# xflouris/libpll-2

Measured on AMD Instinct MI355X. Metric: M site-CLV-updates/s, higher is better.
Workload: dtype f64; 1 GPU; 4-state DNA GTR+G4, 64-taxon balanced tree, 100k sites, tips set with pll_set_tip_states (device reads 1-byte codes: tip x tip / tip x inner kernels at the leaves); sites_per_gpu=100000, ops_per_traversal=62, states=4, taxa=64, step=pll_update_partials(full traversal) + pll_compute_edge_loglikelihood, driver=C loop over the two C-ABI calls (csrc/workload/step_loop.c), parallelism=1 GPU

## Files before the change

libpll-2_amd/csrc/hip/chain_plan.h:

```cpp
#pragma once
struct ChainLaunchRec
{
  unsigned first_head, nchains;
  unsigned variant;
};

struct ChainPlan
{
  std::vector<pllgpu_op_t> key;
  unsigned long long epoch = 0;
  unsigned entries = 0;
  std::vector<CCLaunch> cc;
  std::vector<CC16Launch> cc16;
  std::vector<ChainLaunchRec> stages;
  std::vector<ChainHead> heads;
  std::vector<ChainStepLoad> loads;
  std::vector<ChainStepOp> sops;
  std::vector<unsigned> head_top_clv;
  std::vector<int> head_top_scaler;
  std::vector<unsigned char> head_variant;
  bool in_kernarg = false;
  size_t held_from = 0;
  unsigned launches = 0;
  double bytes = 0.0;
  bool tree = false;
  TreeEnd tree_end[2];
  double tree_bytes = 0.0;
  std::vector<pllgpu_op_t> cherries;
};

static void drop_chain_plan(pllgpu_ctx *c)
{
  if (c->pending_plan == c->plan) c->pending_plan = nullptr;
  delete c->plan;
  c->plan = nullptr;
}

static void chain_steps_on_device(const pllgpu_ctx *c, const ChainPlan &pl, const ChainStepLoad *&lp, const ChainStepOp *&op)
{
  const unsigned char *base = c->chain_dev.p;
  const size_t heads_bytes = pl.heads.size() * sizeof(ChainHead), loads_bytes = pl.loads.size() * sizeof(ChainStepLoad);
  lp = reinterpret_cast<const ChainStepLoad *>(base + heads_bytes);
  op = reinterpret_cast<const ChainStepOp *>(base + heads_bytes + loads_bytes);
}

static void launch_chain_heads(pllgpu_ctx *c, const ChainPlan &pl, unsigned first_head, unsigned nchains, unsigned variant)
{
  const unsigned tiles = (pl.entries + 63) / 64;
  dim3 grid(tiles, nchains), block(256);
  if (pl.in_kernarg)
  {
// ... 11 lines not shown
    }
    with_chain_variant(c->gg.scale_mode, variant, [&](auto SMV, auto C0, auto S1, auto C1) {
      hipLaunchKernelGGL((k_partials_dna_chain_pack<SMV(), C0(), S1(), C1()>), grid, block, 0, c->stream, pack, pl.entries);
    });
  }
  else
  {
    const ChainHead *hp = reinterpret_cast<const ChainHead *>(c->chain_dev.p) + first_head;
    const ChainStepLoad *lp;
    const ChainStepOp *op;
    chain_steps_on_device(c, pl, lp, op);
    with_chain_variant(c->gg.scale_mode, variant, [&](auto SMV, auto C0, auto S1, auto C1) {
      hipLaunchKernelGGL((k_partials_dna_chain<SMV(), C0(), S1(), C1()>), grid, block, 0, c->stream, hp, lp, op, pl.entries);
    });
  }
}

static int launch_chain_plan(pllgpu_ctx *c, const ChainPlan &pl, bool hold)
{
  if (hold && pl.tree)
  {
    c->chain_held = c->tree_held = true;
    c->last_launches = 0;
    c->last_bytes = pl.tree_bytes;
    return 0;
  }
  for (const CC16Launch &l : pl.cc16)
    if (int rc = launch_cc16(c, l.pack, l.n, l.entries)) return rc;
  for (const CCLaunch &l : pl.cc)
    if (int rc = launch_cc(c, l.pack, l.n, l.entries, l.lk, CK_FCC)) return rc;
  const size_t upto = hold ? pl.held_from : pl.stages.size();
  for (size_t i = 0; i < upto; ++i) launch_chain_heads(c, pl, pl.stages[i].first_head, pl.stages[i].nchains, pl.stages[i].variant);
  c->chain_held = hold && upto < pl.stages.size();
  c->last_launches = pl.launches - (unsigned)(pl.stages.size() - upto);
  c->last_bytes = pl.bytes;
  return launch_status();
}

static int launch_held_tree_groups(pllgpu_ctx *c, bool lean = false)
{
  if (!c->tree_held || !c->plan) return 0;
  c->tree_held = false;
  const ChainPlan &pl = *c->plan;
  for (const CCLaunch &l : pl.cc)
    if (int rc = launch_cc(c, l.pack, l.n, l.entries, l.lk, CK_FCC, lean)) return rc;
  c->last_launches += (unsigned)pl.cc.size();
  c->last_bytes = pl.bytes;
// ... 180 lines not shown
        if (P.role[j] == Role::Plain && P.absorb[j] && P.pr_of[1 - P.acc_side[j]][j] == (int)i) st = P.chains[P.chain_of[j]].stage;
    if (stage) stage[i] = st;
    if (chain) chain[i] = member ? -1 : (P.form[i] == 2 ? -2 : P.chain_of[i]);
    if (form) form[i] = member ? 3 : P.form[i];
    stages = std::max(stages, st);
  }
  return (int)stages;
}

static bool use_cc16(const pllgpu_ctx *c, unsigned entries, unsigned count)
{
  if (c->fuse_cc16 >= 0) return c->fuse_cc16 != 0;
  return (size_t)entries * count >= (size_t)9000000;
}

constexpr unsigned kTreeMinEntries = 20000;
static bool use_tree(const pllgpu_ctx *c, unsigned entries, unsigned count)
{
  if (count != 62u || !c->defer_tail) return false;
  if (c->fuse_tree >= 0) return c->fuse_tree != 0;
  return entries >= kTreeMinEntries;
}

struct ChainBuild
{
  const pllgpu_op_t *ops;
  const ChainPartition &part;
  std::vector<DevOp> dev;
  unsigned entries, clv_bytes, sc_bytes;

  ChainLeaf leaf(unsigned i, int sd, bool &tip, ChainLeafBytes &lb) const
  {
    ChainLeaf l;
    tip = ops[i].flags & (sd ? PLLGPU_OP_RIGHT_TIP : PLLGPU_OP_LEFT_TIP);
    lb.clv = lb.aux = lb.pad = 0u;
    if (tip)
    {
      l.data = sd ? dev[i].rtip : dev[i].ltip;
      l.scaler = nullptr;
      lb.aux = (entries + 3u) & ~3u;
    }
    else
    {
      l.data = sd ? dev[i].right : dev[i].left;
      l.scaler = sd ? dev[i].rscaler : dev[i].lscaler;
      lb.clv = clv_bytes;
// ... 97 lines not shown
}

static void choose_held_stage(const pllgpu_ctx *c, ChainPlan *pl)
{
  if (pl->held_from == (size_t)-1) pl->held_from = pl->stages.size();
  unsigned held_chains = 0;
  for (size_t i = pl->held_from; i < pl->stages.size(); ++i) held_chains += pl->stages[i].nchains;
  if (held_chains > 2 || (c->geo.sites + 63) / 64 > 4096u) pl->held_from = pl->stages.size();
  unsigned tail_steps = 0, tail_heads = 0;
  for (size_t i = pl->held_from; i < pl->stages.size(); ++i)
    for (unsigned h = pl->stages[i].first_head; h < pl->stages[i].first_head + pl->stages[i].nchains; ++h, ++tail_heads)
      tail_steps += pl->heads[h].nsteps + 1;
  if (tail_heads && tail_steps + (2u - std::min(tail_heads, 2u)) > (unsigned)kChainPackSteps) pl->in_kernarg = false;
}

static void plan_tree(const pllgpu_ctx *c, const ChainBuild &b, unsigned count, ChainPlan *pl)
{
  const ChainPartition &part = b.part;
  const pllgpu_op_t *ops = b.ops;
  if (count != 62u || part.groups.size() != 8u || part.chains.size() != 2u || pl->heads.size() != 2u) return;
  if (pl->cc.size() != 1u || pl->cc[0].n != 8u || pl->cc[0].lk != CK_FCC || !pl->cc16.empty()) return;
  if (pl->held_from != 0 || pl->stages.empty()) return;
  std::vector<int> group_of(count, -1);
  for (size_t gi = 0; gi < 8u; ++gi)
  {
    const FusedGroup &g = part.groups[gi];
    if (g.lk != CK_FCC || g.rk != CK_FCC || g.absorbed) return;
    group_of[g.p] = (int)gi;
  }
  unsigned seen = 0;
  for (unsigned k = 0; k < 2u; ++k)
  {
    const unsigned top = part.chains[k].ops[0];
    unsigned h = 0;
    while (h < 2u && (pl->head_top_clv[h] != ops[top].parent_clv || pl->head_top_scaler[h] != ops[top].parent_scaler)) ++h;
    if (h == 2u) return;
    TreeEnd &end = pl->tree_end[h];
    memset(&end, 0, sizeof end);
    to_top(b.dev[top], end.top);
    for (int sd = 0; sd < 2; ++sd)
    {
      if (!part.is_chain_op(top, sd)) return;
      const unsigned mid = (unsigned)part.pr_of[sd][top];
      to_top(b.dev[mid], end.mid[sd]);
      for (int sd2 = 0; sd2 < 2; ++sd2)
      {
        const int pr = part.pr_of[sd2][mid];
        if (pr < 0 || group_of[pr] < 0) return;
        seen |= 1u << group_of[pr];
        end.g[sd * 2 + sd2] = pl->cc[0].pack.g[group_of[pr]];
      }
    }
  }
  if (seen != 0xffu) return;
  for (unsigned i = 0; i < count; ++i)
    if ((ops[i].flags & PLLGPU_OP_LEFT_TIP) && (ops[i].flags & PLLGPU_OP_RIGHT_TIP)) pl->cherries.push_back(ops[i]);
  if (pl->cherries.size() != 32u) return;
  for (unsigned i = 0; i < count; ++i)
  {
    const bool lt = (ops[i].flags & PLLGPU_OP_LEFT_TIP) != 0, rt = (ops[i].flags & PLLGPU_OP_RIGHT_TIP) != 0;
    pl->tree_bytes += (c->lazy_cherries && lt && rt) ? 2.0 * ops[i].parent_entries : op_traffic(c, ops[i], lt, rt);
  }
  pl->tree = true;
}

static int build_chain_plan(pllgpu_ctx *c, const pllgpu_op_t *ops, unsigned count, unsigned entries, ChainPartition &part, bool want_tree,
                            ChainPlan *pl)
{
  const std::vector<PChain> &chains = part.chains;
  ChainBuild b{ops, part, std::vector<DevOp>(count), entries, (unsigned)(clv_elems(c, entries) * sizeof(double)),
               entries * (c->gg.scale_mode == 2 ? 16u : 4u)};
  c->last_bytes = 0.0;
  for (unsigned i = 0; i < count; ++i)
    if (part.role[i] == Role::Plain)
      if (int rc = resolve_op(c, ops[i], b.dev[i])) return rc;
  sort_groups_by_level(part.groups);
  if (int rc = build_cc_launches(c, ops, part.groups, 0, part.groups.size(), pl->cc)) return rc;
  if (int rc = build_cc16_launches(c, ops, part.groups, pl->cc16)) return rc;
  unsigned max_stage = 0;
  for (const PChain &ch : chains) max_stage = std::max(max_stage, ch.stage);
  pl->entries = entries;
  pl->in_kernarg = true;
  pl->held_from = (size_t)-1;
  std::vector<unsigned> variant_of(chains.size());
// ... 81 lines not shown
```

libpll-2_amd/csrc/hip/kernels_dna.h:

```cpp
#pragma once
#include "kernels_common.h"

constexpr unsigned kDnaTile = 16 * 64;

template <bool TIP>
__device__ __forceinline__ void dna_fetch(double (&x)[4], const double *__restrict__ base, unsigned k, unsigned code)
{
  if (TIP)
  {
#pragma unroll
    for (int j = 0; j < 4; ++j) x[j] = (code >> j) & 1u ? 1.0 : 0.0;
  }
  else
  {
#pragma unroll
    for (int j = 0; j < 4; ++j) x[j] = __builtin_nontemporal_load(base + (k * 4 + j) * 64);
  }
}

typedef double dbl2 __attribute__((ext_vector_type(2)));
constexpr unsigned kAosLeft = 1u, kAosRight = 2u, kAosParent = 4u, kStreamLeft = 16u, kStreamRight = 32u;

struct DnaCoop
{
// ... 746 lines not shown
  FOp a, b;
  TOp aa, ab;
  TOp ba, bb;
};

constexpr int kMaxCCGroups = 9;

struct CCPack
{
  CCGroup g[kMaxCCGroups];
};

template <bool STORE = true>
__device__ __forceinline__ void dna_cherry(const TOp &t, size_t off, unsigned n, bool valid, int scale_mode, double (&v)[4][4], uint4 &sc)
{
  double xl[4][4], xr[4][4];
  dna_tip_rows(xl, t.ltip[n]);
  dna_tip_rows(xr, t.rtip[n]);
  int mode;
  dna_combine(t, scale_mode, xl, make_uint4(0, 0, 0, 0), xr, make_uint4(0, 0, 0, 0), v, sc, mode);
  if (STORE) dna_store<true>(t.parent, t.pscaler, off, n, valid, mode, v, sc);
}

template <int KIND, bool STORE_CHERRIES = true>
__device__ __forceinline__ void dna_cc_child(const FOp &pop, bool left_side, const FOp &cop, const TOp &x, const TOp &y, size_t off,
                                             unsigned n, bool valid, int scale_mode, double (&v)[4][4], uint4 &sc)
{
  if (KIND == CK_FCC)
  {
    double vx[4][4], vy[4][4];
    uint4 scx, scy;
    int mode;
    dna_cherry<STORE_CHERRIES>(x, off, n, valid, scale_mode, vx, scx);
    dna_cherry<STORE_CHERRIES>(y, off, n, valid, scale_mode, vy, scy);
    dna_combine(cop, scale_mode, vx, scx, vy, scy, v, sc, mode);
    dna_store<true>(cop.parent, cop.pscaler, off, n, valid, mode, v, sc);
  }
  else
  {
    DnaRaw raw;
    dna_child_load<KIND>(pop, left_side, cop, off, n, raw);
    dna_child_compute<KIND>(pop, left_side, cop, n, scale_mode, raw, v, sc);
  }
}

template <int LK, int RK, bool STORE_CHERRIES = true>
__global__ __launch_bounds__(256) void k_partials_dna_cc(const CCPack pack, unsigned entries, int scale_mode, unsigned tiles_per_wave,
                                                          unsigned stream_parent, unsigned nx, unsigned ny, unsigned xcd_order)
{
  unsigned bx, by;
  if (!xcd_block(nx, ny, xcd_order, bx, by)) return;
  const CCGroup &g = pack.g[by];
  for (unsigned t = 0; t < tiles_per_wave; ++t)
  {
    DnaTile w;
    if (!dna_tile(w, bx, tiles_per_wave, t, entries)) break;
    double va[4][4], vb[4][4], v[4][4];
    uint4 sca, scb, sc;
    int mode;
    dna_cc_child<LK, STORE_CHERRIES>(g.p, true, g.a, g.aa, g.ab, w.off, w.n, w.valid, scale_mode, va, sca);
    dna_cc_child<RK, STORE_CHERRIES>(g.p, false, g.b, g.ba, g.bb, w.off, w.n, w.valid, scale_mode, vb, scb);
    dna_combine(g.p, scale_mode, va, sca, vb, scb, v, sc, mode);
    dna_store_parent(stream_parent != 0, g.p.parent, g.p.pscaler, w.off, w.n, w.valid, mode, v, sc);
  }
}

constexpr int CK_F8 = 7;

struct CC16Group
{
  FOp p;
  CCGroup a, b;
};

constexpr int kMaxCC16Groups = 4;

struct CC16Pack
{
  CC16Group g[kMaxCC16Groups];
};

__device__ __forceinline__ void dna_cc8(const CCGroup &g, size_t off, unsigned n, bool valid, int scale_mode, double (&v)[4][4], uint4 &sc)
{
  double va[4][4], vb[4][4];
// ... 775 lines not shown
{
  TreeEnd end[2];
};
static_assert(sizeof(TreePack) + sizeof(DevEdge) + 12 <= 4000, "k_edge_dna_tree's arguments must fit the kernarg segment");

__device__ __forceinline__ void dna_tree_put(double (*xv)[64], uint4 *xs, unsigned lane, const double (&v)[4][4], uint4 sc)
{
#pragma unroll
  for (int k = 0; k < 4; ++k)
#pragma unroll
    for (int i = 0; i < 4; ++i) xv[k * 4 + i][lane] = v[k][i];
  xs[lane] = sc;
}

__device__ __forceinline__ void dna_tree_get(const double (*xv)[64], const uint4 *xs, unsigned lane, double (&v)[4][4], uint4 &sc)
{
#pragma unroll
  for (int k = 0; k < 4; ++k)
#pragma unroll
    for (int i = 0; i < 4; ++i) v[k][i] = xv[k * 4 + i][lane];
  sc = xs[lane];
}

template <bool STORE_CHERRIES>
__device__ __forceinline__ void dna_cc8_parked(const CCGroup &g, double (*xv)[64], uint4 *xs, unsigned lane, size_t off, unsigned n, bool valid,
                                               int scale_mode, double (&v)[4][4], uint4 &sc)
{
  double vb[4][4], u[4][4];
  uint4 scb, scu;
  int mode;
  dna_cc_child<CK_FCC, STORE_CHERRIES>(g.p, true, g.a, g.aa, g.ab, off, n, valid, scale_mode, v, sc);
  dna_tree_put(xv, xs, lane, v, sc);
  asm volatile("" ::: "memory");
  dna_cc_child<CK_FCC, STORE_CHERRIES>(g.p, false, g.b, g.ba, g.bb, off, n, valid, scale_mode, vb, scb);
  asm volatile("" ::: "memory");
  dna_tree_get(xv, xs, lane, v, sc);
  dna_combine(g.p, scale_mode, v, sc, vb, scb, u, scu, mode);
  dna_store<true>(g.p.parent, g.p.pscaler, off, n, valid, mode, u, scu);
#pragma unroll
  for (int k = 0; k < 4; ++k)
#pragma unroll
    for (int i = 0; i < 4; ++i) v[k][i] = u[k][i];
  sc = scu;
}

__device__ __forceinline__ void dna_tree_up(const TOp &op, const double (*xv)[64], const uint4 *xs, unsigned lane, size_t off, unsigned n, bool valid,
                                            int scale_mode, double (&v)[4][4], uint4 &sc)
{
  double vb[4][4], u[4][4];
  uint4 scb, scu;
  int mode;
  dna_tree_get(xv, xs, lane, vb, scb);
  dna_combine(op, scale_mode, v, sc, vb, scb, u, scu, mode);
  dna_store<true>(op.parent, op.pscaler, off, n, valid, mode, u, scu);
#pragma unroll
  for (int k = 0; k < 4; ++k)
#pragma unroll
    for (int i = 0; i < 4; ++i) v[k][i] = u[k][i];
  sc = scu;
}

template <bool STORE_CHERRIES>
__global__ __launch_bounds__(512) void k_edge_dna_tree(const DevEdge e, const TreePack pack, unsigned entries, int scale_mode, unsigned xcd_order)
{
  __shared__ double xv[8][16][64];
  __shared__ uint4 xs[8][64];
  __shared__ unsigned last;
  __shared__ double ws[4];
  const unsigned ntiles = (entries + 63u) / 64u;
  const unsigned tile = xcd_linear(ntiles, xcd_order);
  if (tile == ~0u) return;
  const unsigned lane = threadIdx.x & 63u;
  const unsigned wave = __builtin_amdgcn_readfirstlane(threadIdx.x >> 6);
  const unsigned n0 = tile * 64u + lane;
  const bool valid = n0 < entries;
  const unsigned n = valid ? n0 : entries - 1;
  const size_t off = (size_t)tile * kDnaTile + lane;
  const TreeEnd &end = pack.end[wave >> 2];
  double v[4][4];
  uint4 sc;
  dna_cc8_parked<STORE_CHERRIES>(end.g[wave & 3u], xv[wave], xs[wave], lane, off, n, valid, scale_mode, v, sc);
  if (wave & 1u) dna_tree_put(xv[wave], xs[wave], lane, v, sc);
  lds_barrier();
  if (wave & 1u) return;
  dna_tree_up(end.mid[(wave >> 1) & 1u], xv[wave + 1u], xs[wave + 1u], lane, off, n, valid, scale_mode, v, sc);
  if (wave & 2u) dna_tree_put(xv[wave], xs[wave], lane, v, sc);
  lds_barrier();
  if (!(wave & 2u)) dna_tree_up(end.top, xv[wave + 2u], xs[wave + 2u], lane, off, n, valid, scale_mode, v, sc);
  if (wave == 4u) dna_tree_put(xv[4], xs[4], lane, v, sc);
  lds_barrier();
  if (wave == 0u)
  {
    double vc[4][4];
    uint4 scc;
    dna_tree_get(xv[4], xs[4], lane, vc, scc);
    cdouble_p pm = as_const(e.mat);
    unsigned rs[4];
    const unsigned scal = dna_site_scalers(e, sc, scc, rs);
    const bool is_site = n0 < e.sites;
    const unsigned ns = is_site ? n0 : e.sites - 1;
    const int inv = e.invariant ? e.invariant[ns] : -1;
    double terma = 0.0, terminv = 0.0;
#pragma unroll
    for (int k = 0; k < 4; ++k)
// ... 21 lines not shown
```

libpll-2_amd/csrc/hip/pllgpu.hip:

```cpp
#include "../../../include/pll_amd_device.h"

#include <hip/hip_runtime.h>

#include <algorithm>
#include <atomic>
#include <chrono>
#include <cmath>
#include <thread>
#include <cstdarg>
#include <cstdio>
#include <cstdlib>
#include <cstring>
#include <functional>
#include <map>
#include <mutex>
#include <type_traits>
#include <vector>

#include "kernels_common.h"
#include "kernels_dna.h"
#include "kernels_generic.h"
#include "kernels_deriv.h"
#include "kernels_mfma.h"
#include "kernels_mfma_wide.h"
// ... 125 lines not shown
  void release()
  {
    if (p)
    {
      block_give(p, cap * sizeof(T));
      ++*t_epoch;
    }
    p = nullptr;
    cap = 0;
  }
};

constexpr size_t kResultBytes = (8 + 4 * 64) * sizeof(double);
constexpr unsigned kAscOff = 8;
constexpr unsigned kRepHostCap = 1u << 16;
constexpr unsigned char kMap8 = 1, kMap32 = 2;

struct RellState
{
  DevBuf<unsigned long long> cdf;
  bool stale = true;
  unsigned long long total = 0, not_one = 0;
};

struct pllgpu_ctx
{
  unsigned long long alloc_epoch = 1;
  BlockPool pool;
  pllgpu_geometry_t geo;
  int device = 0;
  hipStream_t stream = nullptr;
  bool own_stream = false;
  hipEvent_t ev0 = nullptr, ev1 = nullptr;

  GenGeo gg;
  int ich = 0;
  bool dna_fast = false;
  bool use_mfma = false;
  int mfma_ng = 16;
  unsigned mfma_wide = 1;
  bool mfma_pad = false;
  unsigned xcd_order = 1;
  bool tiled = false;
  DevBuf<double> scratch;
  size_t pm_stride = 0;
  unsigned span = 0;
// ... 64 lines not shown
  std::vector<unsigned char> stage8;
  unsigned last_launches = 0;
  unsigned long long rep_ops_total = 0, rep_launches_total = 0;
  unsigned long long rep_calls_total = 0;
  double last_bytes = 0.0;
  bool no_tip_columns = false;
  bool tt_stream = true;
  bool no_par_lds = false;
  bool no_coop_fetch = false;
  size_t stream_parent_bytes = (size_t)256 << 20;
  bool defer_tail = false;
  std::vector<pllgpu_op_t> deferred;
  bool fuse_cc = false;
  int fuse_cc16 = -1;
  int fuse_tree = -1;
  bool fuse_gg = true;
  bool fuse = false;
  bool chains = false;
  bool any_aos = false;
  struct ChainPlan *plan = nullptr;
  bool chain_held = false;
  bool tree_held = false;
  bool lazy_cherries = true;
  std::vector<pllgpu_op_t> pending;
  const struct ChainPlan *pending_plan = nullptr;
  DevBuf<double> pending_mats;
  bool pending_mats_kept = false;
  DevBuf<unsigned char> chain_dev;
  unsigned long long maps_epoch = 1;
  unsigned long long maps_version = 1;
  std::vector<unsigned char> map_widened;
  std::vector<struct LevelPlan *> level_plans;
  struct LevelPlan *recording = nullptr;
  int launch_rc = 0;
  int fenced = 0;
  unsigned long long plan_stamp = 0;
  unsigned long long plan_replays = 0;
  bool plan_cache = true;
  DevBuf<unsigned char> cherry_bits;
  struct CherrySlot
  {
    unsigned long long lver = 0, rver = 0, maps = 0;
  };
  std::map<unsigned long long, unsigned> cherry_slot_of;
  std::vector<CherrySlot> cherry_slot;
  std::vector<unsigned long long> pm_version;
  unsigned tip_ncodes = 0;
// ... 135 lines not shown
  c->fuse = c->dna_fast;
  if (const char *v = getenv("PLL_AMD_NO_FUSE"))
    if (*v && *v != '0') c->fuse = false;
  if (const char *v = getenv("PLL_AMD_TT_STREAM")) c->tt_stream = !(*v == '0');
  if (const char *v = getenv("PLL_AMD_NO_TIP_COLUMNS"))
    if (*v && *v != '0') c->no_tip_columns = true;
  if (const char *v = getenv("PLL_AMD_NO_PARENT_LDS"))
    if (*v && *v != '0') c->no_par_lds = true;
  if (const char *v = getenv("PLL_AMD_NO_COOP_FETCH"))
    if (*v && *v != '0') c->no_coop_fetch = true;
  c->defer_tail = c->dna_fast;
  if (const char *v = getenv("PLL_AMD_NO_TAIL_FUSION"))
    if (*v && *v != '0') c->defer_tail = false;
  c->fuse_cc = c->fuse;
  c->fuse_cc16 = -1;
  if (const char *v16 = getenv("PLL_AMD_FUSE_CC16"))
    if (*v16) c->fuse_cc16 = *v16 != '0' ? 1 : 0;
  c->fuse_tree = -1;
  if (const char *vt = getenv("PLL_AMD_FUSE_TREE"))
    if (*vt) c->fuse_tree = *vt != '0' ? 1 : 0;
  c->lazy_cherries = true;
  if (const char *v = getenv("PLL_AMD_LAZY_CHERRIES"))
    if (*v) c->lazy_cherries = *v != '0';
  if (const char *v = getenv("PLL_AMD_NO_FUSE_CC"))
    if (*v && *v != '0') c->fuse_cc = false;
  c->chains = c->fuse;
  if (const char *v = getenv("PLL_AMD_NO_CHAINS"))
    if (*v && *v != '0') c->chains = false;
  if (const char *v = getenv("PLL_AMD_NO_GENERIC_AOS"))
    if (*v && *v != '0') c->generic_aos = false;
  if (const char *v = getenv("PLL_AMD_FENCED_HANDOFF"))
    if (*v && *v != '0') c->fenced = 1;
  if (const char *v = getenv("PLL_AMD_NO_PLAN_CACHE"))
    if (*v && *v != '0') c->plan_cache = false;
  if (const char *v = getenv("PLL_AMD_NEWTON_BATCH"))
    if (atoi(v) >= 1) c->newton_batch = (unsigned)std::min(atoi(v), PLLGPU_NEWTON_MAX_ITERS);
  if (const char *v = getenv("PLL_AMD_NO_FUSE_GG"))
    if (*v && *v != '0') c->fuse_gg = false;
  if (const char *v = getenv("PLL_AMD_RESAMPLE_SCRATCH"))
    if (atoll(v) >= 1) c->resample_bytes = std::min<size_t>((size_t)atoll(v), PLLGPU_RESAMPLE_MAX_BYTES);
  if (const char *v = getenv("PLL_AMD_RELL_RANGE"))
    if (atoll(v) >= 4) c->rell_range = (unsigned)std::min<long long>(atoll(v) / 4 * 4, kRellRange);
  c->subtrees = c->dna_fast;
  if (const char *v = getenv("PLL_AMD_NO_SUBTREES"))
    if (*v && *v != '0') c->subtrees = false;
  c->tiled = true;
// ... 101 lines not shown
    return nullptr;
  }
  c->own_stream = true;
  memset(c->result_host, 0, 8 * sizeof(double));
  memset(c->rep_host, 0, (kRepHostCap + 2) * sizeof(unsigned));
  c->clv.resize(geo->nodes);
  c->clv_aos.assign(geo->nodes, 0);
  c->scaler.resize(geo->scale_buffers);
  c->tipchars.resize(geo->tips);
  c->site_id.resize(geo->nodes);
  c->id_site.resize(geo->nodes);
  c->site_id8.resize(geo->nodes);
  c->rep_keep.resize(geo->nodes);
  c->map_forms.assign(geo->nodes, 0);
  c->map_widened.assign(geo->nodes, 0);
  c->lent.resize(geo->nodes);
  c->rent.resize(geo->nodes);
  c->rep_left.assign(geo->nodes, -1);
  c->rep_right.assign(geo->nodes, -1);
  c->ids.assign(geo->nodes, 0);
  if (c->pmat.ensure(c->pm_stride * (geo->prob_matrices + 2)) || c->freqs.ensure((size_t)geo->rate_matrices * geo->states_padded) ||
      c->rate_weights.ensure(geo->rate_cats) || c->prop_invar.ensure(geo->rate_matrices) ||
      c->pattern_weights.ensure(geo->sites_alloc) || c->persite.ensure(geo->sites_alloc) ||
      c->block_sums.ensure(4096) || c->counter.ensure(4) || (c->dna_fast && c->lazy_cherries && c->pending_mats.ensure(c->pm_stride * 64u)) || c->rep_sync.ensure((size_t)kRepOps + 1) || c->rep_changed.ensure(1))
  {
    pllgpu_destroy(c);
    return nullptr;
  }
  (void)hipMemsetAsync(c->pmat.p, 0, c->pmat.cap * sizeof(double), c->stream);
  c->pm_version.assign(geo->prob_matrices + 2, 1ull);
  (void)hipMemsetAsync(c->prop_invar.p, 0, c->prop_invar.cap * sizeof(double), c->stream);
  (void)hipMemsetAsync(c->counter.p, 0, c->counter.cap * sizeof(unsigned), c->stream);
  (void)hipMemsetAsync(c->rep_sync.p, 0, c->rep_sync.cap * sizeof(unsigned), c->stream);
  (void)hipMemsetAsync(c->rep_changed.p, 0, sizeof(unsigned), c->stream);
  if (const char *v = getenv("PLL_AMD_REP_WGS")) c->rep_wgs = (unsigned)std::max(0, atoi(v));
  if (const char *v = getenv("PLL_AMD_REP_BITS")) c->rep_bits = !(*v == '0');
  if (const char *v = getenv("PLL_AMD_SUB_PACK_ALWAYS")) c->sub_pack_always = *v && *v != '0';
  if (const char *v = getenv("PLL_AMD_REP_FUSE")) c->rep_fuse = !(*v == '0');
  if (const char *v = getenv("PLL_AMD_PINNED_STAGING")) c->ring_failed = *v == '0';
  if (const char *v = getenv("PLL_AMD_REP_HINTS")) c->rep_hints = !(*v == '0');
  if (const char *v = getenv("PLL_AMD_REP_RANGES")) c->rep_max_ranges = (unsigned)std::max(1, atoi(v));
  return c;
}

static void drop_chain_plan(pllgpu_ctx *c);

extern "C" void pllgpu_destroy(pllgpu_ctx_t *c)
// ... 66 lines not shown
  c->rep_counts.release();
  c->rep_sync.release();
  c->rep_changed.release();
  c->rep_final.release();
  c->rates.release();
  c->diag.release();
  c->newton.release();
  for (auto &b : c->sumtable) b.release();
  c->pattern_weights.release();
  c->invariant.release();
  c->pool.trim(0);
  if (c->result_host) (void)hipHostFree(c->result_host);
  if (c->rep_host) (void)hipHostFree(c->rep_host);
  if (c->ring_host) (void)hipHostFree(c->ring_host);
  if (c->ev0) (void)hipEventDestroy(c->ev0);
  if (c->ev1) (void)hipEventDestroy(c->ev1);
  if (c->own_stream && c->stream) (void)hipStreamDestroy(c->stream);
  delete c;
}

static int flush_deferred(pllgpu_ctx *c, bool keep_pending = false);
static int matrices_change(pllgpu_ctx *c, const unsigned *indices, unsigned first, unsigned count);
static int materialise_pending(pllgpu_ctx *c);
static void set_pending(pllgpu_ctx *c, const struct ChainPlan *pl);
#define CHECK_CTX_KEEP(c)                    \
  if (!(c)) return fail(PLLGPU_EINVAL, "null context"); \
  DeviceScope device_scope_(c);              \
  if (device_scope_.rc) return device_scope_.rc
#define HOLDS_WORK(c) (!(c)->deferred.empty() || (c)->chain_held)
#define CHECK_CTX(c)                                   \
  CHECK_CTX_KEEP(c);                                   \
  if (HOLDS_WORK(c) || !(c)->pending.empty())          \
    if (int rc_ = flush_deferred(c)) return rc_
#define CHECK_CTX_KEEP_PENDING(c)                      \
  CHECK_CTX_KEEP(c);                                   \
  if (HOLDS_WORK(c))                                   \
    if (int rc_ = flush_deferred(c, true)) return rc_

constexpr size_t kRingCap = (size_t)8 << 20, kRingMax = (size_t)2 << 20;

static void ring_drained(pllgpu_ctx *c)
{
  for (const auto &d : c->pending_down) memcpy(d.host, d.ring, d.bytes);
  c->pending_down.clear();
  c->ring_off = 0;
}

// ... 859 lines not shown
{
  const unsigned *indices;
  unsigned first, count;
  bool has(unsigned m) const
  {
    if (!indices) return m - first < count;
    for (unsigned i = 0; i < count; ++i)
      if (indices[i] == m) return true;
    return false;
  }
  bool read_by(const pllgpu_op_t &o) const { return has(o.left_matrix) || has(o.right_matrix); }
};

static bool held_work_reads_matrices(const pllgpu_ctx *c, const MatrixSet &ms)
{
  for (const pllgpu_op_t &o : c->deferred)
    if (ms.read_by(o)) return true;
  if (c->chain_held && c->plan)
    for (const pllgpu_op_t &o : c->plan->key)
      if (ms.read_by(o)) return true;
  return false;
}

static void set_pending(pllgpu_ctx *c, const ChainPlan *pl)
{
  c->pending = pl->cherries;
  c->pending_plan = pl;
  c->pending_mats_kept = false;
}

static void drop_pending(pllgpu_ctx *c)
{
  c->pending.clear();
  c->pending_plan = nullptr;
  c->pending_mats_kept = false;
}

static bool clv_is_pending(const pllgpu_ctx *c, unsigned clv)
{
  for (const pllgpu_op_t &o : c->pending)
    if (o.parent_clv == clv) return true;
  return false;
}

struct MatrixCopies
{
  unsigned short src[2 * 32];
};
__global__ void k_keep_matrices(const double *__restrict__ pmat, double *__restrict__ kept, MatrixCopies mc, unsigned stride)
{
  const double *s = pmat + (size_t)mc.src[blockIdx.x] * stride;
  double *d = kept + (size_t)blockIdx.x * stride;
  for (unsigned i = threadIdx.x; i < stride; i += blockDim.x) d[i] = s[i];
}

static int keep_pending_matrices(pllgpu_ctx *c)
{
  if (c->pending.empty() || c->pending_mats_kept) return 0;
  const unsigned n = (unsigned)c->pending.size();
  MatrixCopies mc;
  if (2u * n > sizeof mc.src / sizeof mc.src[0] || c->geo.prob_matrices > 65535u) return materialise_pending(c);
  for (unsigned i = 0; i < n; ++i)
  {
    mc.src[2 * i] = (unsigned short)c->pending[i].left_matrix;
    mc.src[2 * i + 1] = (unsigned short)c->pending[i].right_matrix;
  }
  if (int rc = c->pending_mats.ensure(c->pm_stride * 2u * n)) return rc;
  hipLaunchKernelGGL(k_keep_matrices, dim3(2u * n), dim3(64), 0, c->stream, c->pmat.p, c->pending_mats.p, mc, (unsigned)c->pm_stride);
  if (int rc = launch_status()) return rc;
  c->pending_mats_kept = true;
  return 0;
}

static int matrices_change(pllgpu_ctx *c, const unsigned *indices, unsigned first, unsigned count)
{
  if (!HOLDS_WORK(c) && c->pending.empty()) return 0;
  const MatrixSet ms{indices, first, count};
  if (HOLDS_WORK(c) && held_work_reads_matrices(c, ms))
    if (int rc = flush_deferred(c, true)) return rc;
  if (!c->pending.empty() && !c->pending_mats_kept)
    for (const pllgpu_op_t &o : c->pending)
      if (ms.read_by(o)) return keep_pending_matrices(c);
  return 0;
}

static int materialise_pending(pllgpu_ctx *c)
{
  if (c->pending.empty()) return 0;
  OpPack pack;
  unsigned nops = 0, maxent = 0;
  auto launch = [&]() -> int {
    if (!nops) return 0;
    if (int rc = launch_partials(c, pack, nops, maxent, 2, false)) return rc;
    ++c->last_launches;
    nops = maxent = 0;
    return 0;
  };
  for (size_t i = 0; i < c->pending.size(); ++i)
  {
    const pllgpu_op_t &o = c->pending[i];
    DevOp &d = pack.ops[nops];
    if (int rc = resolve_op(c, o, d)) return rc;
    if (c->pending_mats_kept)
    {
      d.lmat = c->pending_mats.p + (2 * i) * c->pm_stride;
      d.rmat = c->pending_mats.p + (2 * i + 1) * c->pm_stride;
    }
    maxent = std::max(maxent, o.parent_entries);
    if (++nops == (unsigned)kMaxOpsPerLaunch)
      if (int rc = launch()) return rc;
  }
// ... 287 lines not shown
    sort_groups_by_level(groups);
  unsigned i = 0;
  const unsigned last_level = count ? ops[count - 1].level : 0;
  for (unsigned level = 0; level <= last_level; ++level)
  {
    unsigned j = i;
    while (j < count && ops[j].level == level) ++j;
    if (int rc = launch_plain_packs(c, ops, i, j, role)) return rc;
    const size_t g0 = gi_sorted;
    while (gi_sorted < groups.size() && groups[gi_sorted].level == level) ++gi_sorted;
    if (int rc = launch_cc_groups(c, ops, groups, g0, gi_sorted)) return rc;
    if (int rc = launch_gg_packs(c, ops, groups, g0, gi_sorted)) return rc;
    if (int rc = launch_fused_packs(c, ops, groups, g0, gi_sorted)) return rc;
    i = j;
  }
  return launch_status();
}

extern "C" int pllgpu_update_partials(pllgpu_ctx_t *c, const pllgpu_op_t *ops, unsigned count)
{
  CHECK_CTX_KEEP(c);
  const bool replay = c->plan && c->chains && c->fuse && !c->any_aos && c->plan->epoch == c->alloc_epoch && c->plan->key.size() == count &&
                      memcmp(c->plan->key.data(), ops, count * sizeof(pllgpu_op_t)) == 0;
  if (replay && c->pending_plan == c->plan) drop_pending(c);
  if (HOLDS_WORK(c) || !c->pending.empty())
    if (int rc = flush_deferred(c, replay && c->pending.empty())) return rc;
  if (replay && c->pending_plan == c->plan) drop_pending(c);
  c->last_launches = 0;
  c->last_bytes = 0.0;
  {
    bool used = false;
    if (int rc = try_chain_plan(c, ops, count, used)) return rc;
    if (used) return 0;
    c->last_bytes = 0.0;
  }
  if (c->plan_cache)
  {
    const unsigned long long epoch = c->alloc_epoch;
    for (LevelPlan *lp : c->level_plans)
      if (lp->alloc_epoch == epoch && lp->maps_epoch == c->maps_epoch && lp->key.size() == count &&
          memcmp(lp->key.data(), ops, count * sizeof(pllgpu_op_t)) == 0)
      {
        for (const auto &a : lp->aos) c->clv_aos[a.first] = a.second;
        if (lp->any_aos) c->any_aos = true;
        c->deferred = lp->deferred;
        c->launch_rc = 0;
// ... 60 lines not shown
static int launch_edge_tail(pllgpu_ctx *c, const DevEdge &e, const TailCall &t, unsigned blocks, unsigned tpw)
{
  const bool known = with_kind_pair(
      t.kp, t.kc,
      [&](auto KP, auto KC) {
        hipLaunchKernelGGL((k_edge_dna_tail<KP(), KC()>), dim3(blocks), dim3(256), 0, c->stream, e, t.g, c->gg.scale_mode, tpw);
      },
      KindPair<CK_INNER, CK_FTT>(), KindPair<CK_INNER, CK_FTI>(), KindPair<CK_INNER, CK_FII>(),
      KindPair<CK_FTT, CK_INNER>(), KindPair<CK_FTT, CK_TIP>(), KindPair<CK_FTT, CK_FTT>(), KindPair<CK_FTT, CK_FTI>(), KindPair<CK_FTT, CK_FII>(),
      KindPair<CK_FTI, CK_INNER>(), KindPair<CK_FTI, CK_TIP>(), KindPair<CK_FTI, CK_FTT>(), KindPair<CK_FTI, CK_FTI>(), KindPair<CK_FTI, CK_FII>(),
      KindPair<CK_FII, CK_INNER>(), KindPair<CK_FII, CK_TIP>(), KindPair<CK_FII, CK_FTT>(), KindPair<CK_FII, CK_FTI>(), KindPair<CK_FII, CK_FII>());
  if (!known) return fail(PLLGPU_EINVAL, "no tail kernel for end kinds (%d, %d)", t.kp, t.kc);
  return 0;
}

struct ChainTailCall
{
  ChainHead hp, hc;
  unsigned variant;
  bool in_kernarg;
  ChainPack pack;
  const TreePack *tree = nullptr;
  bool lean = false;
};

static void launch_edge_chain(pllgpu_ctx *c, const DevEdge &e, const ChainTailCall &t)
{
  const ChainPlan &pl = *c->plan;
  dim3 grid((pl.entries + 63) / 64), block(256);
  if (t.tree)
    with_bools(!t.lean, false, [&](auto STORE, auto) {
      hipLaunchKernelGGL(k_edge_dna_tree<STORE()>, xcd_grid(grid.x, 1), dim3(512), 0, c->stream, e, *t.tree, pl.entries, c->gg.scale_mode, c->xcd_order);
    });
  else if (t.in_kernarg)
    with_chain_variant(c->gg.scale_mode, t.variant, [&](auto SMV, auto C0, auto S1, auto C1) {
      hipLaunchKernelGGL((k_edge_dna_chain_pack<SMV(), C0(), S1(), C1()>), grid, block, 0, c->stream, e, t.pack, pl.entries);
    });
  else
  {
    const ChainStepLoad *lp;
    const ChainStepOp *op;
    chain_steps_on_device(c, pl, lp, op);
    with_chain_variant(c->gg.scale_mode, t.variant, [&](auto SMV, auto C0, auto S1, auto C1) {
      hipLaunchKernelGGL((k_edge_dna_chain<SMV(), C0(), S1(), C1()>), grid, block, 0, c->stream, e, t.hp, t.hc, lp, op, pl.entries);
    });
  }
}

static int launch_edge_mfma(pllgpu_ctx *c, DevEdge &e, bool ctip, bool gather)
{
  const pllgpu_geometry_t &g = c->geo;
  const unsigned items = (g.sites + 31) / 32, R = c->gg.R;
  const unsigned max_ib = std::max(1u, 512u / R);
  const unsigned ipw = std::max(1u, (items + 4u * max_ib - 1) / (4u * max_ib));
  const unsigned nib = (items + 4u * ipw - 1) / (4u * ipw);
  const unsigned blocks = nib * R;
// ... 374 lines not shown
    ~SeqScope() { c->seq_override = 0.0; }
  } seq_scope_{c};
  c->seq_override = ed->sequence;
  if (int rc = materialise_if_an_end_is_pending(c, ed, false)) return rc;
  ClaimedWork claimed(c);
  TailCall tail;
  bool use_tail = false;
  int held_p = -1, held_c = -1;
  if (int rc = claim_held_chains(c, ed, claimed, held_p, held_c)) return rc;
  if (int rc = claim_held_ops(c, ed, claimed, tail, use_tail)) return rc;
  DevEdge e;
  if (int rc = build_edge(c, ed, e)) return rc;
  int rc;
  if (held_p >= 0 || held_c >= 0)
  {
    ChainTailCall ct;
    TreePack tp;
    if (claimed.tree)
    {
      tp.end[0] = c->plan->tree_end[held_p];
      tp.end[1] = c->plan->tree_end[held_c];
      ct.tree = &tp;
      ct.lean = c->lazy_cherries;
    }
    else if (int brc = build_chain_tail(c, ed, e, held_p, held_c, ct))
      return brc;
    rc = run_lnl(c, e, ed->child_is_tip != 0, false, ed->freqs_indices, persite_host, lnl_out, ed->device_result, nullptr, &ct);
    if (rc == 0 && ct.lean)
    {
      set_pending(c, c->plan);
    }
  }
  else if (use_tail)
  {
    tail.g.p.left = e.parent;
    tail.g.p.lscaler = e.pscaler;
    tail.g.p.right = e.child;
    tail.g.p.rtip = e.ctip;
    tail.g.p.rscaler = e.cscaler;
    rc = run_lnl(c, e, ed->child_is_tip != 0, false, ed->freqs_indices, persite_host, lnl_out, ed->device_result, &tail);
  }
  else
    return run_lnl(c, e, ed->child_is_tip != 0, ed->gather != 0, ed->freqs_indices, persite_host, lnl_out, ed->device_result);
  if (rc == 0) claimed.disarm();
  return rc;
}

extern "C" int pllgpu_root_loglikelihood(pllgpu_ctx_t *c, unsigned clv, int scaler, unsigned gather,
                                         const unsigned *freqs_indices, double *persite_host, double *lnl_out)
{
  CHECK_CTX(c);
  if (clv >= c->geo.nodes || !c->clv[clv].p) return fail(PLLGPU_EINVAL, "CLV %u unavailable on the device", clv);
  DevEdge e;
// ... 2431 lines not shown
```

Before: 67500 M site-CLV-updates/s.

## Defer storing cherry-group subtree CLVs in fused tree kernel until needed

Adds a 'deep' lazy mode for the fused whole-tree edge kernel. On replayed traversals it stores only the top CLVs and skips writing the cherry, child and group-parent CLVs of the eight fused cherry-cherry groups. The skipped ops are recorded as pending subtrees and recomputed by a CC launch only if something later needs them. This cuts global memory writes on the steady-state loop, at the cost of extra bookkeeping and a recompute path with a larger kept-matrix buffer when the pending work is materialised.

```diff
diff --git a/libpll-2_amd/csrc/hip/chain_plan.h b/libpll-2_amd/csrc/hip/chain_plan.h
--- a/libpll-2_amd/csrc/hip/chain_plan.h
+++ b/libpll-2_amd/csrc/hip/chain_plan.h
@@ -27,6 +27,8 @@
   TreeEnd tree_end[2];
   double tree_bytes = 0.0;
   std::vector<pllgpu_op_t> cherries;
+  std::vector<pllgpu_op_t> subtrees;
+  double tree_bytes_deep = 0.0;
 };
 
 static void drop_chain_plan(pllgpu_ctx *c)
@@ -84,7 +86,7 @@
   {
     c->chain_held = c->tree_held = true;
     c->last_launches = 0;
-    c->last_bytes = pl.tree_bytes;
+    c->last_bytes = c->tree_deep ? pl.tree_bytes_deep : pl.tree_bytes;
     return 0;
   }
   for (const CC16Launch &l : pl.cc16)
@@ -311,6 +313,13 @@
   return entries >= kTreeMinEntries;
 }
 
+static bool use_deep_tree(const pllgpu_ctx *c, unsigned entries)
+{
+  if (!c->lazy_cherries) return false;
+  if (c->lazy_subtrees >= 0) return c->lazy_subtrees != 0;
+  return entries >= kTreeMinEntries;
+}
+
 struct ChainBuild
 {
   const pllgpu_op_t *ops;
@@ -454,11 +463,13 @@
   if (pl->cc.size() != 1u || pl->cc[0].n != 8u || pl->cc[0].lk != CK_FCC || !pl->cc16.empty()) return;
   if (pl->held_from != 0 || pl->stages.empty()) return;
   std::vector<int> group_of(count, -1);
+  std::vector<char> in_group(count, 0);
   for (size_t gi = 0; gi < 8u; ++gi)
   {
     const FusedGroup &g = part.groups[gi];
     if (g.lk != CK_FCC || g.rk != CK_FCC || g.absorbed) return;
     group_of[g.p] = (int)gi;
+    in_group[g.a] = in_group[g.b] = 1;
   }
   unsigned seen = 0;
   for (unsigned k = 0; k < 2u; ++k)
@@ -488,10 +499,16 @@
   for (unsigned i = 0; i < count; ++i)
     if ((ops[i].flags & PLLGPU_OP_LEFT_TIP) && (ops[i].flags & PLLGPU_OP_RIGHT_TIP)) pl->cherries.push_back(ops[i]);
   if (pl->cherries.size() != 32u) return;
+  for (size_t gi = 0; gi < 8u; ++gi)
+  {
+    const FusedGroup &g = part.groups[gi];
+    for (int i : {g.aa, g.ab, g.a, g.ba, g.bb, g.b, (int)g.p}) pl->subtrees.push_back(ops[i]);
+  }
   for (unsigned i = 0; i < count; ++i)
   {
     const bool lt = (ops[i].flags & PLLGPU_OP_LEFT_TIP) != 0, rt = (ops[i].flags & PLLGPU_OP_RIGHT_TIP) != 0;
     pl->tree_bytes += (c->lazy_cherries && lt && rt) ? 2.0 * ops[i].parent_entries : op_traffic(c, ops[i], lt, rt);
+    pl->tree_bytes_deep += (lt && rt) ? 2.0 * ops[i].parent_entries : group_of[i] >= 0 || in_group[i] ? 0.0 : op_traffic(c, ops[i], lt, rt);
   }
   pl->tree = true;
 }
diff --git a/libpll-2_amd/csrc/hip/kernels_dna.h b/libpll-2_amd/csrc/hip/kernels_dna.h
--- a/libpll-2_amd/csrc/hip/kernels_dna.h
+++ b/libpll-2_amd/csrc/hip/kernels_dna.h
@@ -792,7 +792,14 @@
   if (STORE) dna_store<true>(t.parent, t.pscaler, off, n, valid, mode, v, sc);
 }
 
-template <int KIND, bool STORE_CHERRIES = true>
+enum class TreeStores
+{
+  All,
+  NoCherries,
+  TopsOnly
+};
+
+template <int KIND, TreeStores ST = TreeStores::All>
 __device__ __forceinline__ void dna_cc_child(const FOp &pop, bool left_side, const FOp &cop, const TOp &x, const TOp &y, size_t off,
                                              unsigned n, bool valid, int scale_mode, double (&v)[4][4], uint4 &sc)
 {
@@ -801,10 +808,10 @@
     double vx[4][4], vy[4][4];
     uint4 scx, scy;
     int mode;
-    dna_cherry<STORE_CHERRIES>(x, off, n, valid, scale_mode, vx, scx);
-    dna_cherry<STORE_CHERRIES>(y, off, n, valid, scale_mode, vy, scy);
+    dna_cherry<ST == TreeStores::All>(x, off, n, valid, scale_mode, vx, scx);
+    dna_cherry<ST == TreeStores::All>(y, off, n, valid, scale_mode, vy, scy);
     dna_combine(cop, scale_mode, vx, scx, vy, scy, v, sc, mode);
-    dna_store<true>(cop.parent, cop.pscaler, off, n, valid, mode, v, sc);
+    if (ST != TreeStores::TopsOnly) dna_store<true>(cop.parent, cop.pscaler, off, n, valid, mode, v, sc);
   }
   else
   {
@@ -828,8 +835,9 @@
     double va[4][4], vb[4][4], v[4][4];
     uint4 sca, scb, sc;
     int mode;
-    dna_cc_child<LK, STORE_CHERRIES>(g.p, true, g.a, g.aa, g.ab, w.off, w.n, w.valid, scale_mode, va, sca);
-    dna_cc_child<RK, STORE_CHERRIES>(g.p, false, g.b, g.ba, g.bb, w.off, w.n, w.valid, scale_mode, vb, scb);
+    constexpr TreeStores ST = STORE_CHERRIES ? TreeStores::All : TreeStores::NoCherries;
+    dna_cc_child<LK, ST>(g.p, true, g.a, g.aa, g.ab, w.off, w.n, w.valid, scale_mode, va, sca);
+    dna_cc_child<RK, ST>(g.p, false, g.b, g.ba, g.bb, w.off, w.n, w.valid, scale_mode, vb, scb);
     dna_combine(g.p, scale_mode, va, sca, vb, scb, v, sc, mode);
     dna_store_parent(stream_parent != 0, g.p.parent, g.p.pscaler, w.off, w.n, w.valid, mode, v, sc);
   }
@@ -1651,21 +1659,21 @@
   sc = xs[lane];
 }
 
-template <bool STORE_CHERRIES>
+template <TreeStores ST>
 __device__ __forceinline__ void dna_cc8_parked(const CCGroup &g, double (*xv)[64], uint4 *xs, unsigned lane, size_t off, unsigned n, bool valid,
                                                int scale_mode, double (&v)[4][4], uint4 &sc)
 {
   double vb[4][4], u[4][4];
   uint4 scb, scu;
   int mode;
-  dna_cc_child<CK_FCC, STORE_CHERRIES>(g.p, true, g.a, g.aa, g.ab, off, n, valid, scale_mode, v, sc);
+  dna_cc_child<CK_FCC, ST>(g.p, true, g.a, g.aa, g.ab, off, n, valid, scale_mode, v, sc);
   dna_tree_put(xv, xs, lane, v, sc);
   asm volatile("" ::: "memory");
-  dna_cc_child<CK_FCC, STORE_CHERRIES>(g.p, false, g.b, g.ba, g.bb, off, n, valid, scale_mode, vb, scb);
+  dna_cc_child<CK_FCC, ST>(g.p, false, g.b, g.ba, g.bb, off, n, valid, scale_mode, vb, scb);
   asm volatile("" ::: "memory");
   dna_tree_get(xv, xs, lane, v, sc);
   dna_combine(g.p, scale_mode, v, sc, vb, scb, u, scu, mode);
-  dna_store<true>(g.p.parent, g.p.pscaler, off, n, valid, mode, u, scu);
+  if (ST != TreeStores::TopsOnly) dna_store<true>(g.p.parent, g.p.pscaler, off, n, valid, mode, u, scu);
 #pragma unroll
   for (int k = 0; k < 4; ++k)
 #pragma unroll
@@ -1689,7 +1697,7 @@
   sc = scu;
 }
 
-template <bool STORE_CHERRIES>
+template <TreeStores ST>
 __global__ __launch_bounds__(512) void k_edge_dna_tree(const DevEdge e, const TreePack pack, unsigned entries, int scale_mode, unsigned xcd_order)
 {
   __shared__ double xv[8][16][64];
@@ -1708,7 +1716,7 @@
   const TreeEnd &end = pack.end[wave >> 2];
   double v[4][4];
   uint4 sc;
-  dna_cc8_parked<STORE_CHERRIES>(end.g[wave & 3u], xv[wave], xs[wave], lane, off, n, valid, scale_mode, v, sc);
+  dna_cc8_parked<ST>(end.g[wave & 3u], xv[wave], xs[wave], lane, off, n, valid, scale_mode, v, sc);
   if (wave & 1u) dna_tree_put(xv[wave], xs[wave], lane, v, sc);
   lds_barrier();
   if (wave & 1u) return;
diff --git a/libpll-2_amd/csrc/hip/pllgpu.hip b/libpll-2_amd/csrc/hip/pllgpu.hip
--- a/libpll-2_amd/csrc/hip/pllgpu.hip
+++ b/libpll-2_amd/csrc/hip/pllgpu.hip
@@ -171,6 +171,8 @@
   bool stale = true;
   unsigned long long total = 0, not_one = 0;
 };
+
+constexpr unsigned kMaxPending = 56;
 
 struct pllgpu_ctx
 {
@@ -281,7 +283,10 @@
   bool chain_held = false;
   bool tree_held = false;
   bool lazy_cherries = true;
+  int lazy_subtrees = -1;
+  bool tree_deep = false;
   std::vector<pllgpu_op_t> pending;
+  bool pending_deep = false;
   const struct ChainPlan *pending_plan = nullptr;
   DevBuf<double> pending_mats;
   bool pending_mats_kept = false;
@@ -463,6 +468,9 @@
   c->lazy_cherries = true;
   if (const char *v = getenv("PLL_AMD_LAZY_CHERRIES"))
     if (*v) c->lazy_cherries = *v != '0';
+  c->lazy_subtrees = -1;
+  if (const char *v = getenv("PLL_AMD_LAZY_SUBTREES"))
+    if (*v) c->lazy_subtrees = *v != '0' ? 1 : 0;
   if (const char *v = getenv("PLL_AMD_NO_FUSE_CC"))
     if (*v && *v != '0') c->fuse_cc = false;
   c->chains = c->fuse;
@@ -610,7 +618,7 @@
   if (c->pmat.ensure(c->pm_stride * (geo->prob_matrices + 2)) || c->freqs.ensure((size_t)geo->rate_matrices * geo->states_padded) ||
       c->rate_weights.ensure(geo->rate_cats) || c->prop_invar.ensure(geo->rate_matrices) ||
       c->pattern_weights.ensure(geo->sites_alloc) || c->persite.ensure(geo->sites_alloc) ||
-      c->block_sums.ensure(4096) || c->counter.ensure(4) || (c->dna_fast && c->lazy_cherries && c->pending_mats.ensure(c->pm_stride * 64u)) || c->rep_sync.ensure((size_t)kRepOps + 1) || c->rep_changed.ensure(1))
+      c->block_sums.ensure(4096) || c->counter.ensure(4) || (c->dna_fast && c->lazy_cherries && c->pending_mats.ensure(c->pm_stride * 2u * kMaxPending)) || c->rep_sync.ensure((size_t)kRepOps + 1) || c->rep_changed.ensure(1))
   {
     pllgpu_destroy(c);
     return nullptr;
@@ -723,7 +731,7 @@
 static int flush_deferred(pllgpu_ctx *c, bool keep_pending = false);
 static int matrices_change(pllgpu_ctx *c, const unsigned *indices, unsigned first, unsigned count);
 static int materialise_pending(pllgpu_ctx *c);
-static void set_pending(pllgpu_ctx *c, const struct ChainPlan *pl);
+static void set_pending(pllgpu_ctx *c, const struct ChainPlan *pl, bool deep = false);
 #define CHECK_CTX_KEEP(c)                    \
   if (!(c)) return fail(PLLGPU_EINVAL, "null context"); \
   DeviceScope device_scope_(c);              \
@@ -1629,9 +1637,10 @@
   return false;
 }
 
-static void set_pending(pllgpu_ctx *c, const ChainPlan *pl)
-{
-  c->pending = pl->cherries;
+static void set_pending(pllgpu_ctx *c, const ChainPlan *pl, bool deep)
+{
+  c->pending = deep ? pl->subtrees : pl->cherries;
+  c->pending_deep = deep;
   c->pending_plan = pl;
   c->pending_mats_kept = false;
 }
@@ -1639,6 +1648,7 @@
 static void drop_pending(pllgpu_ctx *c)
 {
   c->pending.clear();
+  c->pending_deep = false;
   c->pending_plan = nullptr;
   c->pending_mats_kept = false;
 }
@@ -1652,7 +1662,7 @@
 
 struct MatrixCopies
 {
-  unsigned short src[2 * 32];
+  unsigned short src[2 * kMaxPending];
 };
 __global__ void k_keep_matrices(const double *__restrict__ pmat, double *__restrict__ kept, MatrixCopies mc, unsigned stride)
 {
@@ -1691,9 +1701,44 @@
   return 0;
 }
 
+static int materialise_pending_groups(pllgpu_ctx *c)
+{
+  const size_t ngroups = c->pending.size() / 7u;
+  if (c->pending.size() != ngroups * 7u || ngroups == 0 || ngroups > (size_t)kMaxCCGroups) return fail(PLLGPU_ERUNTIME, "pending groups out of shape");
+  CCPack pack;
+  memset(&pack, 0, sizeof pack);
+  for (size_t gi = 0; gi < ngroups; ++gi)
+  {
+    CCGroup &cg = pack.g[gi];
+    TOp *tops[7] = {&cg.aa, &cg.ab, nullptr, &cg.ba, &cg.bb, nullptr, nullptr};
+    FOp *fops[7] = {nullptr, nullptr, &cg.a, nullptr, nullptr, &cg.b, &cg.p};
+    for (size_t k = 0; k < 7u; ++k)
+    {
+      const size_t i = gi * 7u + k;
+      DevOp d;
+      if (int rc = resolve_op(c, c->pending[i], d)) return rc;
+      if (c->pending_mats_kept)
+      {
+        d.lmat = c->pending_mats.p + (2 * i) * c->pm_stride;
+        d.rmat = c->pending_mats.p + (2 * i + 1) * c->pm_stride;
+      }
+      if (tops[k])
+        to_top(d, *tops[k]);
+      else
+        to_fop(d, *fops[k]);
+    }
+  }
+  if (int rc = launch_cc(c, pack, (unsigned)ngroups, c->pending[0].parent_entries, CK_FCC, CK_FCC)) return rc;
+  ++c->last_launches;
+  if (int rc = launch_status()) return rc;
+  drop_pending(c);
+  return 0;
+}
+
 static int materialise_pending(pllgpu_ctx *c)
 {
   if (c->pending.empty()) return 0;
+  if (c->pending_deep) return materialise_pending_groups(c);
   OpPack pack;
   unsigned nops = 0, maxent = 0;
   auto launch = [&]() -> int {
@@ -2027,6 +2072,7 @@
   CHECK_CTX_KEEP(c);
   const bool replay = c->plan && c->chains && c->fuse && !c->any_aos && c->plan->epoch == c->alloc_epoch && c->plan->key.size() == count &&
                       memcmp(c->plan->key.data(), ops, count * sizeof(pllgpu_op_t)) == 0;
+  c->tree_deep = replay && c->pending_plan == c->plan && !c->pending.empty() && c->plan->tree && use_deep_tree(c, c->plan->entries);
   if (replay && c->pending_plan == c->plan) drop_pending(c);
   if (HOLDS_WORK(c) || !c->pending.empty())
     if (int rc = flush_deferred(c, replay && c->pending.empty())) return rc;
@@ -2133,6 +2179,7 @@
   ChainPack pack;
   const TreePack *tree = nullptr;
   bool lean = false;
+  bool deep = false;
 };
 
 static void launch_edge_chain(pllgpu_ctx *c, const DevEdge &e, const ChainTailCall &t)
@@ -2140,9 +2187,17 @@
   const ChainPlan &pl = *c->plan;
   dim3 grid((pl.entries + 63) / 64), block(256);
   if (t.tree)
-    with_bools(!t.lean, false, [&](auto STORE, auto) {
-      hipLaunchKernelGGL(k_edge_dna_tree<STORE()>, xcd_grid(grid.x, 1), dim3(512), 0, c->stream, e, *t.tree, pl.entries, c->gg.scale_mode, c->xcd_order);
-    });
+  {
+    auto go = [&](auto ST) {
+      hipLaunchKernelGGL(k_edge_dna_tree<ST()>, xcd_grid(grid.x, 1), dim3(512), 0, c->stream, e, *t.tree, pl.entries, c->gg.scale_mode, c->xcd_order);
+    };
+    if (t.deep)
+      go(std::integral_constant<TreeStores, TreeStores::TopsOnly>());
+    else if (t.lean)
+      go(std::integral_constant<TreeStores, TreeStores::NoCherries>());
+    else
+      go(std::integral_constant<TreeStores, TreeStores::All>());
+  }
   else if (t.in_kernarg)
     with_chain_variant(c->gg.scale_mode, t.variant, [&](auto SMV, auto C0, auto S1, auto C1) {
       hipLaunchKernelGGL((k_edge_dna_chain_pack<SMV(), C0(), S1(), C1()>), grid, block, 0, c->stream, e, t.pack, pl.entries);
@@ -2563,13 +2618,14 @@
       tp.end[1] = c->plan->tree_end[held_c];
       ct.tree = &tp;
       ct.lean = c->lazy_cherries;
+      ct.deep = ct.lean && c->tree_deep;
     }
     else if (int brc = build_chain_tail(c, ed, e, held_p, held_c, ct))
       return brc;
     rc = run_lnl(c, e, ed->child_is_tip != 0, false, ed->freqs_indices, persite_host, lnl_out, ed->device_result, nullptr, &ct);
     if (rc == 0 && ct.lean)
     {
-      set_pending(c, c->plan);
+      set_pending(c, c->plan, ct.deep);
     }
   }
   else if (use_tail)
```

Result: faster. 79380 M site-CLV-updates/s, median of 6 (+17.6%).
